# Zilong-Li/BaseVarC

Measured on AMD Instinct MI355X. Metric: sites/sec at N=1e6 samples; achieved HBM GB/s vs roofline, higher is better.
Workload: dtype f64

## Files before the change

### basevarc_amd/csrc/bvc_context.hip

```cpp
#include <cmath>
#include <cstdlib>
#include <cstring>
#include <mutex>
#include <new>

#include "bvc_ctx.h"

hipError_t sync_streams(bvc_ctx *ctx)
{
    hipError_t first = hipSuccess;
    for (hipStream_t s : streams_of(ctx)) {
        const hipError_t e = hipStreamSynchronize(s);
        if (first == hipSuccess) first = e;
    }
    for (bool &p : ctx->em_pending) p = false;
    return first;
}

int drain_on_error(bvc_ctx *ctx, int code)
{
    (void)sync_streams(ctx);
    (void)hipGetLastError();
    return code;
}
// ... 158 lines not shown
    if (hipSetDevice(device) != hipSuccess) { delete ctx; return BVC_ERR_DEVICE; }
    QualLut lut;
    for (int q = 0; q < 128; ++q) {
        const double eps = std::exp(-0.23025850929940458 * q);
        lut.a[q] = 1.0 - eps;
        lut.e[q] = eps / 3.0;
        lut.log_e[q] = std::log(lut.e[q]);
        lut.log_a[q] = std::log(lut.a[q]);
    }
    lut.e_empty = 0.25;
    if (hipMalloc(reinterpret_cast<void **>(&ctx->d_lut), sizeof(QualLut)) != hipSuccess ||
        hipMemcpy(ctx->d_lut, &lut, sizeof(QualLut), hipMemcpyHostToDevice) != hipSuccess) {
        (void)hipGetLastError();
        if (ctx->d_lut) (void)hipFree(ctx->d_lut);
        delete ctx;
        return BVC_ERR_ALLOC;
    }
    int prio_least = 0, prio_greatest = 0;
    if (hipDeviceGetStreamPriorityRange(&prio_least, &prio_greatest) != hipSuccess) { (void)hipGetLastError(); prio_least = 0; }
    const int side_prio = env_int("BVC_SIDE_PRIORITY", 0, 1, 1) ? prio_least : 0;
    bool ok = hipStreamCreateWithFlags(&ctx->own_stream, hipStreamDefault) == hipSuccess &&
              hipEventCreateWithFlags(&ctx->ev_wait, hipEventBlockingSync | hipEventDisableTiming) == hipSuccess &&
              hipStreamCreateWithPriority(&ctx->side, hipStreamNonBlocking, side_prio) == hipSuccess &&
              hipStreamCreateWithPriority(&ctx->side_b, hipStreamNonBlocking, side_prio) == hipSuccess &&
              hipStreamCreateWithPriority(&ctx->side_c, hipStreamNonBlocking, side_prio) == hipSuccess &&
              hipStreamCreateWithFlags(&ctx->copy, hipStreamNonBlocking) == hipSuccess &&
              hipMalloc(reinterpret_cast<void **>(&ctx->d_grp_scratch), kGroupScratchWords * sizeof(int64_t)) == hipSuccess &&
              hipMalloc(reinterpret_cast<void **>(&ctx->d_sink), 256) == hipSuccess;
    for (int b = 0; b < bvc_ctx::kRing && ok; ++b)
        ok = hipEventCreateWithFlags(&ctx->ev_hist_done[b], hipEventDisableTiming) == hipSuccess &&
             hipEventCreateWithFlags(&ctx->ev_em_done[b], hipEventDisableTiming) == hipSuccess;
    for (int b = 0; b < 2 && ok; ++b) ok = hipEventCreateWithFlags(&ctx->ev_upload[b], hipEventDisableTiming) == hipSuccess;
    for (int b = 0; b < 2 && ok; ++b) ok = hipEventCreateWithFlags(&ctx->ev_set_free[b], hipEventDisableTiming) == hipSuccess;
    if (!ok) { (void)hipGetLastError(); bvc_destroy(ctx); return BVC_ERR_DEVICE; }
    ctx->stream = ctx->own_stream;
    *out = ctx;
    return BVC_OK;
}

void *bvc_host_alloc(size_t bytes)
{
    void *p = nullptr;
    if (bytes == 0) bytes = 1;
    if (hipHostMalloc(&p, bytes, hipHostMallocPortable) != hipSuccess) { (void)hipGetLastError(); return nullptr; }
    std::lock_guard<std::mutex> g(g_pinned_mu);
    g_pinned.push_back({static_cast<const char *>(p), bytes});
    return p;
}

void bvc_host_free(void *p)
{
    if (!p) return;
    {
        std::lock_guard<std::mutex> g(g_pinned_mu);
        for (size_t i = 0; i < g_pinned.size(); ++i)
            if (g_pinned[i].first == p) { g_pinned.erase(g_pinned.begin() + (long)i); break; }
    }
    (void)hipHostFree(p);
}

void bvc_destroy(bvc_ctx *ctx)
{
    if (!ctx) return;
    (void)hipSetDevice(ctx->device);
    (void)sync_streams(ctx);
    for (hipStream_t s : {ctx->side, ctx->side_b, ctx->side_c, ctx->copy, ctx->own_stream})
        if (s) (void)hipStreamDestroy(s);
    if (ctx->ev_wait) (void)hipEventDestroy(ctx->ev_wait);
    for (int b = 0; b < bvc_ctx::kRing; ++b) {
        if (ctx->ev_hist_done[b]) (void)hipEventDestroy(ctx->ev_hist_done[b]);
        if (ctx->ev_em_done[b]) (void)hipEventDestroy(ctx->ev_em_done[b]);
    }
    for (int b = 0; b < 2; ++b) {
        if (ctx->ev_upload[b]) (void)hipEventDestroy(ctx->ev_upload[b]);
        if (ctx->ev_set_free[b]) (void)hipEventDestroy(ctx->ev_set_free[b]);
    }
    for (auto &t : ctx->ev_pending) give_back(ctx, t);
    for (auto e : ctx->ev_pool) (void)hipEventDestroy(e);
    if (ctx->d_lut) (void)hipFree(ctx->d_lut);
    if (ctx->d_grp_scratch) (void)hipFree(ctx->d_grp_scratch);
    if (ctx->d_sink) (void)hipFree(ctx->d_sink);
    if (ctx->h_up) (void)hipHostFree(ctx->h_up);
    if (ctx->h_down) (void)hipHostFree(ctx->h_down);
    delete ctx;
}

const char *bvc_last_error(const bvc_ctx *ctx) { return ctx ? ctx->err.c_str() : "null context"; }

int bvc_set_stream(bvc_ctx *ctx, void *hip_stream)
{
    if (!ctx) return BVC_ERR_ARG;
    BVC_HIP(ctx, hipSetDevice(ctx->device));
    BVC_HIP(ctx, sync_streams(ctx));
    ctx->stream = reinterpret_cast<hipStream_t>(hip_stream);
    return BVC_OK;
}

int bvc_synchronize(bvc_ctx *ctx)
{
    if (!ctx) return BVC_ERR_ARG;
    BVC_HIP(ctx, hipSetDevice(ctx->device));
    BVC_HIP(ctx, sync_streams(ctx));
    return BVC_OK;
}

int bvc_set_overlap(bvc_ctx *ctx, int on)
{
    if (!ctx) return BVC_ERR_ARG;
    BVC_HIP(ctx, hipSetDevice(ctx->device));
// ... 100 lines not shown
```

### basevarc_amd/csrc/bvc_ctx.h

```cpp
#pragma once
#include <hip/hip_runtime.h>

#include <array>
#include <cstring>
#include <string>
#include <vector>

#include "bvc_internal.h"

using namespace bvc;

#pragma GCC visibility push(hidden)

struct DevBuf {
    char *p = nullptr;
    size_t cap = 0;
    DevBuf() = default;
    DevBuf(const DevBuf &) = delete;
    DevBuf &operator=(const DevBuf &) = delete;
    ~DevBuf() { if (p) (void)hipFree(p); }
};

struct PileupState {
    DevBuf text, meta, out, called;
// ... 6 lines not shown
        int64_t entries = 0, obs = 0, indels = 0;
        int64_t text_bytes = 0, indel_bytes = 0;
        bool on_device_text = false;
    } tile;
};

struct bvc_ctx {
    int device = -1;
    hipStream_t stream = nullptr;
    hipStream_t own_stream = nullptr;
    hipEvent_t ev_wait = nullptr;
    QualLut *d_lut = nullptr;
    static constexpr int kRing = 4;
    DevBuf d_cnt[kRing];
    bool overlap = false;
    hipStream_t side = nullptr;
    hipStream_t side_b = nullptr, side_c = nullptr;
    unsigned side_flip = 0;
    int flip = 0;
    hipEvent_t ev_hist_done[kRing] = {};
    hipEvent_t ev_em_done[kRing] = {};
    bool em_pending[kRing] = {};
    DevBuf d_grp[kRing];
    DevBuf d_em[kRing + 1];
    DevBuf d_emg[kRing];
    uint32_t *d_sink = nullptr;
    DevBuf d_acc;
    DevBuf d_grp_labels;
    int64_t *d_grp_scratch = nullptr;
    DevBuf d_stage[2];
    hipStream_t copy = nullptr;
    hipEvent_t ev_upload[2] = {nullptr, nullptr};
    hipEvent_t ev_set_free[2] = {nullptr, nullptr};
    PileupState pile;
    char *h_up = nullptr, *h_down = nullptr;
    size_t up_cap = 0, down_cap = 0;
    LaunchState ls;
    bool profiling = false;
    std::vector<hipEvent_t> ev_pool;
    struct Triple { hipEvent_t a, b, c, d; int64_t sites; };
    std::vector<Triple> ev_pending;
    bvc_profile prof{};
    std::string err;
};

struct RingSlot {
    uint32_t *counts = nullptr, *grp = nullptr;
    void *em = nullptr, *emg = nullptr;
};

inline int fail(bvc_ctx *ctx, int code, const char *what, hipError_t e = hipSuccess)
{
    if (ctx) {
        ctx->err = what;
        if (e != hipSuccess) { ctx->err += ": "; ctx->err += hipGetErrorString(e); }
    }
    return code;
}

inline hipError_t wait_stream(bvc_ctx *ctx)
{
    hipError_t e = hipEventRecord(ctx->ev_wait, ctx->stream);
    return e == hipSuccess ? hipEventSynchronize(ctx->ev_wait) : e;
}

#define BVC_HIP(ctx, call)                                                         \
// ... 62 lines not shown
    std::vector<Out> outs;
    explicit PinIO(bvc_ctx *c) : ctx(c) {}
    static size_t al(size_t n) { return (n + 63) & ~(size_t)63; }
    int reserve(size_t up_bytes, size_t down_bytes)
    {
        auto grow = [&](char **buf, size_t *cap, size_t need) -> int {
            if (need <= *cap) return BVC_OK;
            if (*buf) {
                if (wait_stream(ctx) != hipSuccess) return fail(ctx, BVC_ERR_DEVICE, "wait before growing a pinned buffer");
                (void)hipHostFree(*buf);
                *buf = nullptr; *cap = 0;
            }
            const size_t want = need + need / 4 + 4096;
            if (hipHostMalloc(reinterpret_cast<void **>(buf), want, hipHostMallocDefault) != hipSuccess) {
                (void)hipGetLastError();
                return fail(ctx, BVC_ERR_ALLOC, "pinned host allocation failed");
            }
            *cap = want;
            return BVC_OK;
        };
        int rc = grow(&ctx->h_up, &ctx->up_cap, up_bytes);
        return rc == BVC_OK ? grow(&ctx->h_down, &ctx->down_cap, down_bytes) : rc;
    }
    hipError_t h2d(void *dev, const void *host, size_t n)
    {
        if (n == 0) return hipSuccess;
        if (in_pinned(host, n)) return hipMemcpyAsync(dev, host, n, hipMemcpyHostToDevice, ctx->stream);
        if (up_used + n > ctx->up_cap) return hipErrorOutOfMemory;
        char *p = ctx->h_up + up_used;
        std::memcpy(p, host, n);
        up_used += al(n);
        return hipMemcpyAsync(dev, p, n, hipMemcpyHostToDevice, ctx->stream);
    }
    hipError_t d2h(void *host, const void *dev, size_t n)
    {
        if (n == 0) return hipSuccess;
        if (down_used + n > ctx->down_cap) return hipErrorOutOfMemory;
        char *p = ctx->h_down + down_used;
        down_used += al(n);
        outs.push_back(Out{host, p, n});
        return hipMemcpyAsync(p, dev, n, hipMemcpyDeviceToHost, ctx->stream);
    }
    void deliver() { for (auto const &o : outs) std::memcpy(o.dst, o.src, o.n); outs.clear(); }
};

inline int check_common(bvc_ctx *ctx, int64_t n_sites, const void *a, const void *b, const void *c, const void *d)
{
    if (!ctx) return BVC_ERR_ARG;
    if (n_sites < 0) return fail(ctx, BVC_ERR_ARG, "n_sites < 0");
    if (n_sites > 0 && (!a || !b || !c || !d)) return fail(ctx, BVC_ERR_ARG, "null data pointer");
    if (n_sites > (int64_t)0x7FFFFFFF / 64) return fail(ctx, BVC_ERR_ARG, "too many sites in one call (split the tile)");
    BVC_HIP(ctx, hipSetDevice(ctx->device));
    return BVC_OK;
}

inline int check_dense(bvc_ctx *ctx, int64_t n_sites, int64_t n_samples, int64_t row_stride, const void *a, const void *b, const void *c,
                       const void *d)
{
    const int rc = check_common(ctx, n_sites, a, b, c, d);
    if (rc != BVC_OK) return rc;
    return n_samples >= 0 && row_stride >= n_samples ? BVC_OK : fail(ctx, BVC_ERR_ARG, "need 0 <= n_samples <= row_stride");
}

inline int check_offsets_host(bvc_ctx *ctx, int64_t n_sites, const int64_t *offsets)
{
    bool ok = offsets[0] == 0;
    for (int64_t s = 0; s < n_sites && ok; ++s) ok = offsets[s + 1] >= offsets[s];
    return ok ? BVC_OK : fail(ctx, BVC_ERR_ARG, "offsets must start at 0 and be non-decreasing");
}

inline int check_n_groups(bvc_ctx *ctx, int32_t n_groups)
{
    return n_groups >= 1 && n_groups <= BVC_MAX_GROUPS ? BVC_OK : fail(ctx, BVC_ERR_ARG, "n_groups must be 1..32");
// ... 11 lines not shown
```

### basevarc_amd/csrc/bvc_internal.h

```cpp
#pragma once
#include <hip/hip_runtime.h>
#include <stdint.h>

#include <vector>

#include "../../include/bvc.h"

namespace bvc {

struct LaunchState {
    int n_cu = 256;
    int em_waves_per_cu = 0;
    int em_wpb = 4;
    int hist_split = 0;
    int host_chunk_kib = 1 << 19;
    int em_streams = 0;
    int group_pipe = 1;
    int group_log2c = -1;
    int group_big_lds = 1;
    int group_h16 = 0;
    int em_engine = 0;
    int em_tiny_regions = 0;
    int csr_scatter_max = 64;
    int em_prune = 1;
// ... 77 lines not shown
                              int8_t *bases, int8_t *quals, int8_t *ref_base);

struct PileupTile {
    const uint8_t *text = nullptr;
    bool bin = false;
    const uint32_t *line_start = nullptr;
    const int32_t *sample0 = nullptr, *n_in_batch = nullptr;
    int32_t n_batches = 0, n_pos = 0;
    int32_t line_stride = 0;
    const int32_t *n_pos_dev = nullptr;
    int64_t n_lines_cap = 0;
    uint32_t *line_words = nullptr;
    uint32_t *status = nullptr;
    int64_t *entry_off = nullptr, *obs_off = nullptr, *totals = nullptr;
    bvc_pileup_entry *entries = nullptr;
    int32_t *samples = nullptr;
    int8_t *obs_base = nullptr, *obs_qual = nullptr;
    const uint8_t *group_of_sample = nullptr;
    int64_t n_samples = 0;
    int32_t n_groups = 0;
    uint8_t *obs_label = nullptr;
    int32_t *tally = nullptr;
    bvc_pileup_indel *indels = nullptr;
    uint32_t indel_cap = 0;
};
struct bvc_pileup_region { uint32_t start, len, left_src, left_len; };
hipError_t launch_region_carry(hipStream_t stream, const uint8_t *old_text, uint8_t *text, const bvc_pileup_region *regions, int32_t n_batches);
hipError_t launch_region_index(hipStream_t stream, const PileupTile &P, const bvc_pileup_region *regions, const uint32_t *seg_base,
                               int64_t n_segments, uint32_t *seg_nl, int32_t *lines, int32_t max_pos);
hipError_t launch_region_ends(hipStream_t stream, const PileupTile &P, uint32_t *ends);
hipError_t launch_indel_text(hipStream_t stream, const PileupTile &P, uint8_t *dst, uint32_t dst_cap, uint32_t *used);
hipError_t launch_called_scan(hipStream_t stream, const PileupTile &P, const bvc_site_result *results, int64_t *called_off);
hipError_t launch_called_gather(hipStream_t stream, const PileupTile &P, const int64_t *called_off, bvc_pileup_entry *out_entries,
                                int32_t *out_samples);
hipError_t launch_pileup_count(hipStream_t stream, const PileupTile &P);
hipError_t launch_pileup_write(hipStream_t stream, const PileupTile &P, uint32_t carry_in);
hipError_t launch_hist_csr_groups(LaunchState &st, hipStream_t stream, int64_t n_sites, const int64_t *offsets, const int8_t *bases,
                                  const int8_t *quals, const int32_t *sample_of_obs, const uint8_t *group_of_sample, int64_t n_samples,
                                  int n_groups, uint32_t *counts);
hipError_t launch_hist_csr_labels(LaunchState &st, hipStream_t stream, int64_t n_sites, const int64_t *offsets, const uint8_t *obs,
                                  const uint8_t *quals, const uint8_t *group_of_obs, int n_groups, uint32_t *counts);

hipError_t launch_counts_add(hipStream_t stream, int64_t n_words, uint32_t *dst, const uint32_t *src);
hipError_t launch_hist_csr_scatter(const LaunchState &st, hipStream_t stream, int64_t n_sites, const int64_t *offsets, const uint8_t *obs,
                                   const uint8_t *quals, const uint8_t *group_of_obs, int n_groups, int64_t max_len, uint32_t *counts);
hipError_t launch_hist_csr_add(LaunchState &st, hipStream_t stream, int64_t n_sites, const int64_t *offsets, const uint8_t *obs,
                               const uint8_t *quals, const uint8_t *group_of_obs, int n_groups, int64_t min_len, uint32_t *counts);

constexpr int kStatsMaxLog2c = 4;
constexpr int kSiteStatsTrip = 4096;
hipError_t launch_site_stats(LaunchState &st, hipStream_t stream, int64_t n_sites, const int64_t *offsets, const bvc_pileup_entry *entries,
                             const int8_t *ref_base, const bvc_site_result *results, bvc_site_stats *stats);

hipError_t launch_inflate(hipStream_t stream, const uint8_t *comp, const bvc_bgzf_block *blocks, int64_t n_blocks, uint8_t *out, uint32_t *status);

#ifdef BVC_CHECK_LDS
hipError_t debug_read_inflate(uint32_t *out8, bool reset);
hipError_t debug_read_pileup(uint32_t *out8, bool reset);
hipError_t debug_read_site_stats(uint32_t *out8, bool reset);
hipError_t debug_read_hist(uint32_t *out8, bool reset);
hipError_t debug_read_wave_engine(uint32_t *out8, bool reset);
hipError_t debug_read_items(uint32_t *out8, bool reset);
#endif

}
```

### basevarc_amd/csrc/bvc_pileup.hip

```cpp
#include "bvc_ctx.h"

extern "C" {

int bvc_inflate_blocks(bvc_ctx *ctx, const uint8_t *comp, int64_t comp_bytes, const bvc_bgzf_block *blocks, int64_t n_blocks,
                       uint8_t *out, int64_t out_bytes, uint32_t *status, uint32_t flags)
{
    if (!ctx) return BVC_ERR_ARG;
    if (n_blocks < 0 || comp_bytes < 0 || out_bytes < 0) return fail(ctx, BVC_ERR_ARG, "negative size");
    if (n_blocks == 0) return BVC_OK;
    if (!comp || !blocks || !status || (!out && out_bytes > 0)) return fail(ctx, BVC_ERR_ARG, "null data pointer");
    BVC_HIP(ctx, hipSetDevice(ctx->device));
    if (flags & BVC_PTR_DEVICE) {
        BVC_HIP(ctx, launch_inflate(ctx->stream, comp, blocks, n_blocks, out, status));
        return BVC_OK;
    }
    for (int64_t i = 0; i < n_blocks; ++i) {
        const bvc_bgzf_block &b = blocks[i];
        if (b.comp_off < 0 || b.comp_len < 0 || b.comp_off + b.comp_len > comp_bytes || b.isize < 0 || b.isize > 65536 || b.out_off < 0 ||
            b.out_off + b.isize > out_bytes)
            return fail(ctx, BVC_ERR_ARG, "block outside its buffer");
    }
    uint8_t *d_c, *d_o; bvc_bgzf_block *d_b; uint32_t *d_s;
    int rc = carve(ctx, ctx->d_stage[0], 256, [&](Layout &L) {
        d_c = L.take<uint8_t>((size_t)comp_bytes, 16);
// ... 188 lines not shown
            d_reg = L.take<bvc_pileup_region>(nb);
            d_sb = L.take<uint32_t>(nb + 1);
            d_sn = L.take<uint32_t>(segs, 4);
            d_lines = L.take<int32_t>(nb, 4);
            d_ends = L.take<uint32_t>(nb, 4);
        });
    if (rc != BVC_OK) return rc;
    uint8_t *text_out = reinterpret_cast<uint8_t *>(pile.pz_text[nw].p);
    P.text = text_out;
    int32_t *d_T = reinterpret_cast<int32_t *>(reinterpret_cast<char *>(P.status) + 128);
    P.n_pos_dev = d_T;
    PinIO io(ctx);
    rc = io.reserve((n_blocks > 0 && in_pinned(comp, (size_t)comp_bytes) ? 0 : (size_t)comp_bytes) + (size_t)n_blocks * sizeof(bvc_bgzf_block) +
                        nb * (sizeof(bvc_pileup_region) + 12) + 1024,
                    (size_t)n_blocks * 4 + nb * 8 + 1024);
    if (rc != BVC_OK) return rc;
    BVC_HIP_D(ctx, hipMemsetAsync(P.status, 0, clear, ctx->stream));
    std::vector<uint32_t> bst((size_t)n_blocks);
    std::vector<uint32_t> ends(nb);
    uint32_t st[8] = {0, 0, 0, 0, 0, 0, 0, 0};
    int64_t tot[2] = {0, 0};
    int32_t Tgot = 0;
    if (nb > 0) {
        if (n_blocks > 0) {
            BVC_HIP_D(ctx, io.h2d(pile.pz_comp.p, comp, (size_t)comp_bytes));
            BVC_HIP_D(ctx, io.h2d(d_blk, blk.data(), (size_t)n_blocks * sizeof(bvc_bgzf_block)));
        }
        BVC_HIP_D(ctx, io.h2d(d_reg, reg.data(), nb * sizeof(bvc_pileup_region)));
        BVC_HIP_D(ctx, io.h2d(d_sb, seg_base.data(), (nb + 1) * 4));
        BVC_HIP_D(ctx, io.h2d(d_s0, sample0, nb * 4));
        BVC_HIP_D(ctx, io.h2d(d_nib, n_in_batch, nb * 4));
        BVC_HIP_D(ctx, launch_region_carry(ctx->stream, reinterpret_cast<const uint8_t *>(pile.pz_text[pile.pz_cur].p), text_out, d_reg,
                                           n_batches));
        if (n_blocks > 0)
            BVC_HIP_D(ctx, launch_inflate(ctx->stream, reinterpret_cast<const uint8_t *>(pile.pz_comp.p), d_blk, n_blocks, text_out, d_bst));
        BVC_HIP_D(ctx, launch_region_index(ctx->stream, P, d_reg, d_sb, (int64_t)segs, d_sn, d_lines, max_positions));
        BVC_HIP_D(ctx, launch_region_ends(ctx->stream, P, d_ends));
        BVC_HIP_D(ctx, launch_pileup_count(ctx->stream, P));
        if (n_blocks > 0) BVC_HIP_D(ctx, io.d2h(bst.data(), d_bst, (size_t)n_blocks * 4));
        BVC_HIP_D(ctx, io.d2h(lines_of_batch, d_lines, nb * 4));
        BVC_HIP_D(ctx, io.d2h(ends.data(), d_ends, nb * 4));
        BVC_HIP_D(ctx, io.d2h(&Tgot, d_T, 4));
    }
    BVC_HIP_D(ctx, io.d2h(st, P.status, sizeof st));
    BVC_HIP_D(ctx, io.d2h(tot, P.totals, sizeof tot));
    BVC_HIP_D(ctx, wait_stream(ctx));
    io.deliver();
    for (int64_t i = 0; i < n_blocks; ++i)
        if (bst[(size_t)i] != 0) {
            pile.left_len.assign(nb, 0u);
            return fail(ctx, BVC_ERR_DATA, bst[(size_t)i] == 10 ? "a BGZF block of a temp batch fails its CRC32"
                                                                : "a BGZF block of a temp batch is not valid deflate of its ISIZE bytes");
        }
    for (size_t b = 0; b < nb; ++b) { pile.left_src[b] = ends[b]; pile.left_len[b] = region_end[b] - ends[b]; }
    pile.pz_cur = nw;
    P.n_pos = Tgot; P.n_pos_dev = nullptr;
    pile.tile.text_bytes = (int64_t)text_bytes;
    pile.tile.on_device_text = true;
    *n_positions = Tgot;
    if (Tgot == 0) return BVC_OK;
    if (st[0] != 0) return BVC_PILEUP_IRREGULAR;
    pile.tile.entries = tot[0]; pile.tile.obs = tot[1]; pile.tile.indels = st[1]; pile.tile.indel_bytes = st[4];
    pile.tile.begun = true;
    *n_entries = tot[0]; *n_indels = st[1]; *indel_text_bytes = st[4];
    return BVC_OK;
}

int bvc_pileup_text(bvc_ctx *ctx, char *text, int64_t text_cap, int64_t *text_bytes_needed, uint32_t *line_start)
{
    if (!ctx || !text_bytes_needed) return BVC_ERR_ARG;
    const PileupState::Tile &tile = ctx->pile.tile;
    if (!tile.on_device_text) return fail(ctx, BVC_ERR_ARG, "bvc_pileup_text without a tile from bvc_pileup_begin_bgzf");
    *text_bytes_needed = tile.text_bytes;
    if (!text) return BVC_OK;
    if (text_cap < tile.text_bytes || !line_start) return fail(ctx, BVC_ERR_ARG, "text buffer too small / null line table");
    BVC_HIP(ctx, hipSetDevice(ctx->device));
    const PileupTile &P = tile.P;
    if (tile.text_bytes) BVC_HIP(ctx, hipMemcpyAsync(text, P.text, (size_t)tile.text_bytes, hipMemcpyDeviceToHost, ctx->stream));
    if (P.n_batches > 0)
        BVC_HIP(ctx, hipMemcpy2DAsync(line_start, (size_t)(P.n_pos + 1) * 4, P.line_start, (size_t)P.line_stride * 4, (size_t)(P.n_pos + 1) * 4,
                                      (size_t)P.n_batches, hipMemcpyDeviceToHost, ctx->stream));
    BVC_HIP(ctx, wait_stream(ctx));
    return BVC_OK;
}

static int pileup_finish_impl(bvc_ctx *ctx, const int8_t *ref_base, double min_af, const uint8_t carry_in[5], uint8_t carry_out[5],
                              const uint8_t *group_of_sample, int64_t n_samples, int32_t n_groups,
                              int64_t *entry_off, int32_t *tally, int64_t *called_off, int64_t called_cap, bvc_pileup_entry *entries,
                              int32_t *samples, bvc_pileup_indel *indels, char *indel_text, bvc_site_result *results,
                              bvc_group_result *grp_results, bvc_site_stats *stats)
{
    if (!ctx) return BVC_ERR_ARG;
    PileupState &pile = ctx->pile;
    PileupState::Tile &tile = pile.tile;
    if (!tile.begun) return fail(ctx, BVC_ERR_ARG, "bvc_pileup_finish without a bvc_pileup_begin that returned BVC_OK");
    if (tile.on_device_text && tile.indels > 0 && !indel_text) return fail(ctx, BVC_ERR_ARG, "indel_text is needed: the tile's text is on the device only");
    tile.begun = false;
    PileupTile &P = tile.P;
    const int64_t T = P.n_pos, n_e = tile.entries, n_o = tile.obs, n_i = tile.indels, n_it = tile.indel_bytes;
    if (!carry_in || !carry_out || !entry_off) return fail(ctx, BVC_ERR_ARG, "null pointer");
    if (T > 0 && (!ref_base || !tally || !results)) return fail(ctx, BVC_ERR_ARG, "null pointer");
    const bool called_only = called_off != nullptr;
    if ((n_e > 0 && !called_only && (!entries || !samples)) || (n_i > 0 && !indels)) return fail(ctx, BVC_ERR_ARG, "null pointer");
    if (called_only && (called_cap < 0 || (called_cap > 0 && (!entries || !samples)))) return fail(ctx, BVC_ERR_ARG, "null pointer");
    if (n_groups < 0 || n_groups > BVC_MAX_GROUPS) return fail(ctx, BVC_ERR_ARG, "n_groups must be 0..32");
    if (n_groups > 0 && (!grp_results || n_samples < 0 || (n_samples > 0 && !group_of_sample))) return fail(ctx, BVC_ERR_ARG, "null group pointer");
    BVC_HIP(ctx, hipSetDevice(ctx->device));
    int8_t *d_ref; bvc_site_result *d_res; uint8_t *d_g, *d_itext; bvc_group_result *d_gres; int64_t *d_called_off; bvc_site_stats *d_stats;
    int rc = carve(ctx, pile.out, 256, [&](Layout &L) {
        P.entries = L.take<bvc_pileup_entry>((size_t)n_e, 16);
        P.samples = L.take<int32_t>((size_t)n_e, 16);
        P.obs_base = L.take<int8_t>((size_t)n_o, 16);
        P.obs_qual = L.take<int8_t>((size_t)n_o, 16);
        P.obs_label = L.take<uint8_t>((size_t)(n_groups ? n_o : 0), 16);
        P.indels = L.take<bvc_pileup_indel>((size_t)n_i, 16);
        d_ref = L.take<int8_t>((size_t)T, 16);
        d_res = L.take<bvc_site_result>((size_t)T);
        d_g = L.take<uint8_t>((size_t)(n_groups ? n_samples : 0), 16);
        d_gres = L.take<bvc_group_result>((size_t)T * (size_t)n_groups);
        d_itext = L.take<uint8_t>((size_t)(indel_text ? n_it : 0), 16);
        d_called_off = L.take<int64_t>(called_only ? (size_t)(T + 1) : 0);
        d_stats = L.take<bvc_site_stats>(stats ? (size_t)T : 0);
    });
    if (rc != BVC_OK) return rc;
    P.indel_cap = (uint32_t)n_i;
    P.group_of_sample = d_g; P.n_samples = n_groups ? n_samples : 0; P.n_groups = n_groups;
    const uint32_t cin = (uint32_t)(carry_in[0] & 7u) | ((uint32_t)(carry_in[4] & 1u) << 3) | 0x80u | ((uint32_t)carry_in[1] << 8) |
                         ((uint32_t)carry_in[2] << 16) | ((uint32_t)carry_in[3] << 24);
    uint32_t cout = cin;
    PinIO io(ctx);
    rc = io.reserve((size_t)T + (size_t)(n_groups > 0 ? n_samples : 0) + 1024,
                    (size_t)T * (sizeof(bvc_site_result) + 32 * 4 + 8 + (size_t)n_groups * sizeof(bvc_group_result)) +
                        (size_t)(called_only ? 0 : n_e) * (sizeof(bvc_pileup_entry) + 4) + (called_only ? (size_t)(T + 1) * 8 : 0) +
                        (size_t)n_i * sizeof(bvc_pileup_indel) + (size_t)n_it + (stats ? (size_t)T * sizeof(bvc_site_stats) : 0) + 4096);
    if (rc != BVC_OK) return rc;
    if (T > 0) {
        BVC_HIP_D(ctx, io.h2d(d_ref, ref_base, (size_t)T));
        if (n_groups > 0 && n_samples > 0) BVC_HIP_D(ctx, io.h2d(d_g, group_of_sample, (size_t)n_samples));
        if ((int64_t)P.n_pos * P.n_batches > 0) BVC_HIP_D(ctx, launch_pileup_write(ctx->stream, P, cin));
        if (n_groups > 0)
            rc = run_csr_labels_device(ctx, T, P.obs_off, reinterpret_cast<const uint8_t *>(P.obs_base),
                                       reinterpret_cast<const uint8_t *>(P.obs_qual), P.obs_label, d_ref, min_af, n_groups, d_res, d_gres);
        else
            rc = run_csr_device(ctx, T, P.obs_off, P.obs_base, P.obs_qual, d_ref, min_af, nullptr, nullptr, d_res);
        if (rc == BVC_OK) rc = join_side(ctx);
        if (rc != BVC_OK) return drain_on_error(ctx, rc);
        if (stats) BVC_HIP_D(ctx, launch_site_stats(ctx->ls, ctx->stream, T, P.entry_off, P.entries, d_ref, d_res, d_stats));
        BVC_HIP_D(ctx, io.d2h(results, d_res, (size_t)T * sizeof(bvc_site_result)));
        if (stats) BVC_HIP_D(ctx, io.d2h(stats, d_stats, (size_t)T * sizeof(bvc_site_stats)));
        if (n_groups > 0)
            BVC_HIP_D(ctx, io.d2h(grp_results, d_gres, (size_t)T * (size_t)n_groups * sizeof(bvc_group_result)));
        BVC_HIP_D(ctx, io.d2h(tally, P.tally, (size_t)T * 32 * 4));
        if (n_e && !called_only) {
            BVC_HIP_D(ctx, io.d2h(entries, P.entries, (size_t)n_e * sizeof(bvc_pileup_entry)));
            BVC_HIP_D(ctx, io.d2h(samples, P.samples, (size_t)n_e * 4));
        }
        if (called_only) {
            BVC_HIP_D(ctx, launch_called_scan(ctx->stream, P, d_res, d_called_off));
            BVC_HIP_D(ctx, io.d2h(called_off, d_called_off, (size_t)(T + 1) * 8));
        }
        if (n_i && indel_text) {
            BVC_HIP_D(ctx, launch_indel_text(ctx->stream, P, d_itext, (uint32_t)n_it, P.status + 5));
            if (n_it) BVC_HIP_D(ctx, io.d2h(indel_text, d_itext, (size_t)n_it));
        }
        if (n_i) BVC_HIP_D(ctx, io.d2h(indels, P.indels, (size_t)n_i * sizeof(bvc_pileup_indel)));
        if ((int64_t)P.n_pos * P.n_batches > 0) BVC_HIP_D(ctx, io.d2h(&cout, P.status + 3, 4));
    }
    BVC_HIP_D(ctx, io.d2h(entry_off, P.entry_off, (size_t)(T + 1) * 8));
    BVC_HIP_D(ctx, wait_stream(ctx));
    io.deliver();
    if (called_only && T == 0) called_off[0] = 0;
    if (called_only && T > 0 && called_off[T] > 0) {
        const int64_t n_c = called_off[T];
        if (n_c > called_cap) return fail(ctx, BVC_ERR_ARG, "called_cap is smaller than the entries of the called positions (n_entries of the begin call always suffices)");
        bvc_pileup_entry *d_ce; int32_t *d_cs;
        rc = carve(ctx, pile.called, 0, [&](Layout &L) {
            d_ce = L.take<bvc_pileup_entry>((size_t)n_c);
            d_cs = L.take<int32_t>((size_t)n_c);
        });
        if (rc != BVC_OK) return rc;
        io.down_used = 0;
        rc = io.reserve(0, (size_t)n_c * (sizeof(bvc_pileup_entry) + 4) + 4096);
        if (rc != BVC_OK) return rc;
        BVC_HIP_D(ctx, launch_called_gather(ctx->stream, P, d_called_off, d_ce, d_cs));
        BVC_HIP_D(ctx, io.d2h(entries, d_ce, (size_t)n_c * sizeof(bvc_pileup_entry)));
        BVC_HIP_D(ctx, io.d2h(samples, d_cs, (size_t)n_c * 4));
        BVC_HIP_D(ctx, wait_stream(ctx));
        io.deliver();
    }
    carry_out[0] = (uint8_t)(cout & 7u); carry_out[1] = (uint8_t)(cout >> 8); carry_out[2] = (uint8_t)(cout >> 16);
    carry_out[3] = (uint8_t)(cout >> 24); carry_out[4] = (uint8_t)((cout >> 3) & 1u);
    return BVC_OK;
}

int bvc_pileup_finish(bvc_ctx *ctx, const int8_t *ref_base, double min_af, const uint8_t carry_in[5], uint8_t carry_out[5],
                      const uint8_t *group_of_sample, int64_t n_samples, int32_t n_groups,
                      int64_t *entry_off, int32_t *tally, bvc_pileup_entry *entries, int32_t *samples,
                      bvc_pileup_indel *indels, char *indel_text, bvc_site_result *results, bvc_group_result *grp_results)
{
    return pileup_finish_impl(ctx, ref_base, min_af, carry_in, carry_out, group_of_sample, n_samples, n_groups, entry_off, tally, nullptr, 0,
                              entries, samples, indels, indel_text, results, grp_results, nullptr);
}

int bvc_pileup_finish_called(bvc_ctx *ctx, const int8_t *ref_base, double min_af, const uint8_t carry_in[5], uint8_t carry_out[5],
                             const uint8_t *group_of_sample, int64_t n_samples, int32_t n_groups,
                             int64_t *entry_off, int32_t *tally, int64_t *called_off, int64_t called_cap, bvc_pileup_entry *entries,
                             int32_t *samples, bvc_pileup_indel *indels, char *indel_text, bvc_site_result *results,
                             bvc_group_result *grp_results)
{
    if (ctx && !called_off) return fail(ctx, BVC_ERR_ARG, "null pointer");
    return pileup_finish_impl(ctx, ref_base, min_af, carry_in, carry_out, group_of_sample, n_samples, n_groups, entry_off, tally, called_off,
                              called_cap, entries, samples, indels, indel_text, results, grp_results, nullptr);
}

int bvc_pileup_finish_called_stats(bvc_ctx *ctx, const int8_t *ref_base, double min_af, const uint8_t carry_in[5], uint8_t carry_out[5],
                                   const uint8_t *group_of_sample, int64_t n_samples, int32_t n_groups,
                                   int64_t *entry_off, int32_t *tally, int64_t *called_off, int64_t called_cap, bvc_pileup_entry *entries,
                                   int32_t *samples, bvc_pileup_indel *indels, char *indel_text, bvc_site_result *results,
                                   bvc_group_result *grp_results, bvc_site_stats *stats)
{
    if (ctx && !called_off) return fail(ctx, BVC_ERR_ARG, "null pointer");
// ... 6 lines not shown
```

### basevarc_amd/csrc/inflate_kernel.hip

```cpp
#include <hip/hip_runtime.h>

#ifndef BVC_INFLATE_WINDOW
#define BVC_INFLATE_WINDOW 4096
#endif

#include "bvc_device.h"
#include "bvc_internal.h"

namespace bvc {
namespace {

constexpr uint32_t kWinBytes = BVC_INFLATE_WINDOW, kWinMask = kWinBytes - 1;
constexpr uint32_t kDump = kWinBytes;
constexpr bool kWholeWindow = kWinBytes == 32768;
static_assert((kWinBytes & kWinMask) == 0 && kWinBytes >= 4096 && kWinBytes <= 32768, "the LDS ring: a power of two, 4..32 KiB");
constexpr int kLitBits = 9, kDistBits = 7, kPreBits = 7;
constexpr uint32_t kValid = 0x80000000u;
constexpr uint32_t kKindLiteral = 0u << 24, kKindEnd = 1u << 24, kKindLength = 2u << 24, kKindBad = 3u << 24, kKindMask = 3u << 24;

__device__ const uint16_t kLenBase[29] = {3, 4, 5, 6, 7, 8, 9, 10, 11, 13, 15, 17, 19, 23, 27, 31, 35, 43, 51, 59, 67, 83, 99, 115, 131, 163, 195, 227, 258};
__device__ const uint8_t kLenExtra[29] = {0, 0, 0, 0, 0, 0, 0, 0, 1, 1, 1, 1, 2, 2, 2, 2, 3, 3, 3, 3, 4, 4, 4, 4, 5, 5, 5, 5, 0};
__device__ const uint16_t kDistBase[30] = {1, 2, 3, 4, 5, 7, 9, 13, 17, 25, 33, 49, 65, 97, 129, 193, 257, 385, 513, 769, 1025, 1537, 2049, 3073, 4097, 6145,
                                           8193, 12289, 16385, 24577};
__device__ const uint8_t kDistExtra[30] = {0, 0, 0, 0, 1, 1, 2, 2, 3, 3, 4, 4, 5, 5, 6, 6, 7, 7, 8, 8, 9, 9, 10, 10, 11, 11, 12, 12, 13, 13};
// ... 577 lines not shown
        const uint32_t n = (uint32_t)blocks[blk].isize;
        const uint64_t base = o0 & ~(uint64_t)15;
        const uint32_t span = (uint32_t)(o0 - base) + n;
        const uint32_t per = ((span + kWave - 1) / kWave + 15u) & ~15u;
        const uint64_t lo64 = base + (uint64_t)per * (uint32_t)lane, hi64 = lo64 + per;
        const uint64_t lo = lo64 < o0 ? o0 : (lo64 > o0 + n ? o0 + n : lo64), hi = hi64 < o0 ? o0 : (hi64 > o0 + n ? o0 + n : hi64);
        uint32_t c = 0xFFFFFFFFu;
        uint64_t at = lo;
        while (at < hi && (at & 15u)) { c = tab[(c ^ out[at]) & 255u] ^ (c >> 8); ++at; }
        for (; at + 16 <= hi; at += 16) {
            const uint4 v = *reinterpret_cast<const uint4 *>(out + at);
            const uint32_t w[4] = {v.x, v.y, v.z, v.w};
#pragma unroll
            for (int j = 0; j < 4; ++j)
#pragma unroll
                for (int b = 0; b < 4; ++b) c = tab[(c ^ (w[j] >> (8 * b))) & 255u] ^ (c >> 8);
        }
        for (; at < hi; ++at) c = tab[(c ^ out[at]) & 255u] ^ (c >> 8);
        const uint32_t mine = ~c;
        const uint32_t len = (uint32_t)(hi - lo);
        const uint32_t op_full = crc_shift_op(per);
        uint32_t acc = (uint32_t)__builtin_amdgcn_readlane((int)mine, 0);
        for (int k = 1; k < kWave; ++k) {
            const uint32_t lk = (uint32_t)__shfl((int)len, k, kWave), ck = (uint32_t)__shfl((int)mine, k, kWave);
            if (lk == 0u) continue;
            acc = crc_multmodp(lk == per ? op_full : crc_shift_op(lk), acc) ^ ck;
        }
        if (lane == 0 && acc != blocks[blk].crc32) status[blk] = kErrCrc;
    }
}

}

hipError_t launch_inflate(hipStream_t stream, const uint8_t *comp, const bvc_bgzf_block *blocks, int64_t n_blocks, uint8_t *out, uint32_t *status)
{
    if (n_blocks <= 0) return hipSuccess;
    hipLaunchKernelGGL(inflate_kernel, dim3((unsigned)(n_blocks < 65536 ? n_blocks : 65536)), dim3(kWave), 0, stream, comp, blocks, n_blocks, out, status);
    hipLaunchKernelGGL(crc32_kernel, dim3((unsigned)(n_blocks < 65536 ? n_blocks : 65536)), dim3(kWave), 0, stream, blocks, n_blocks, out, status);
    return hipGetLastError();
}

#ifdef BVC_CHECK_LDS
BVC_DEFINE_DEBUG_READER(debug_read_inflate)
#endif

}
```

### basevarc_amd/csrc/pileup_kernel.hip

```cpp
#include <hip/hip_runtime.h>

#include "bvc_device.h"
#include "bvc_internal.h"

namespace bvc {
namespace {

constexpr int kParseWaves = 4;
constexpr uint32_t kTokValid = 0x80u;

typedef uint32_t u32x4 __attribute__((ext_vector_type(4)));
typedef uint32_t u32x2 __attribute__((ext_vector_type(2)));

__device__ __forceinline__ uint32_t wave_incl_scan(uint32_t v, int lane)
{
#pragma unroll
    for (int d = 1; d < kWave; d <<= 1) {
        const uint32_t u = (uint32_t)__shfl_up((int)v, d, kWave);
        if (lane >= d) v += u;
    }
    return v;
}

__device__ __forceinline__ uint32_t wave_sum(uint32_t v)
// ... 707 lines not shown
    }
}

__global__ __launch_bounds__(1024) void called_scan_kernel(int64_t n_pos, const bvc_site_result *__restrict__ results,
                                                           const int64_t *__restrict__ entry_off, int64_t *__restrict__ called_off)
{
    __shared__ int64_t wave_sum[16];
    __shared__ int64_t running;
    const int lane = threadIdx.x & (kWave - 1), wave = threadIdx.x >> 6;
    if (threadIdx.x == 0) running = 0;
    __syncthreads();
    for (int64_t t0 = 0; t0 < n_pos; t0 += 1024) {
        const int64_t t = t0 + threadIdx.x;
        const int64_t mine = (t < n_pos && results[t].called) ? entry_off[t + 1] - entry_off[t] : 0;
        int64_t incl = mine;
        for (int d = 1; d < kWave; d <<= 1) {
            const int64_t up = __shfl_up(incl, d);
            if (lane >= d) incl += up;
        }
        if (lane == kWave - 1) wave_sum[wave] = incl;
        __syncthreads();
        int64_t before = running;
        for (int w = 0; w < wave; ++w) before += wave_sum[w];
        if (t < n_pos) called_off[t] = before + incl - mine;
        __syncthreads();
        if (threadIdx.x == 1023) running = before + incl;
        __syncthreads();
    }
    if (threadIdx.x == 0) called_off[n_pos] = running;
}

__global__ void called_gather_kernel(int64_t n_pos, const int64_t *__restrict__ entry_off, const int64_t *__restrict__ called_off,
                                     const bvc_pileup_entry *__restrict__ entries, const int32_t *__restrict__ samples,
                                     bvc_pileup_entry *__restrict__ out_entries, int32_t *__restrict__ out_samples)
{
    for (int64_t t = blockIdx.x; t < n_pos; t += gridDim.x) {
        const int64_t at = called_off[t], n = called_off[t + 1] - at, from = entry_off[t];
        for (int64_t i = threadIdx.x; i < n; i += blockDim.x) {
            out_entries[at + i] = entries[from + i];
            out_samples[at + i] = samples[from + i];
        }
    }
}

hipError_t launch_called_scan(hipStream_t stream, const PileupTile &P, const bvc_site_result *results, int64_t *called_off)
{
    hipLaunchKernelGGL(called_scan_kernel, dim3(1), dim3(1024), 0, stream, (int64_t)P.n_pos, results, P.entry_off, called_off);
    return hipGetLastError();
}

hipError_t launch_called_gather(hipStream_t stream, const PileupTile &P, const int64_t *called_off, bvc_pileup_entry *out_entries,
                                int32_t *out_samples)
{
    if (P.n_pos <= 0) return hipSuccess;
    hipLaunchKernelGGL(called_gather_kernel, dim3((unsigned)(P.n_pos < 16384 ? P.n_pos : 16384)), dim3(256), 0, stream, (int64_t)P.n_pos,
                       P.entry_off, called_off, P.entries, P.samples, out_entries, out_samples);
    return hipGetLastError();
}

hipError_t launch_region_carry(hipStream_t stream, const uint8_t *old_text, uint8_t *text, const bvc_pileup_region *regions, int32_t n_batches)
{
    if (n_batches <= 0) return hipSuccess;
    hipLaunchKernelGGL(region_carry_kernel, dim3((unsigned)n_batches), dim3(256), 0, stream, old_text, text, regions);
    return hipGetLastError();
}

hipError_t launch_region_index(hipStream_t stream, const PileupTile &P, const bvc_pileup_region *regions, const uint32_t *seg_base,
                               int64_t n_segments, uint32_t *seg_nl, int32_t *lines, int32_t max_pos)
{
    if (P.n_batches <= 0) return hipSuccess;
    RegionArgs A{};
    A.text = P.text; A.regions = regions; A.seg_base = seg_base; A.n_batches = P.n_batches; A.max_pos = max_pos; A.line_stride = P.line_stride;
    A.seg_nl = seg_nl; A.lines = lines; A.n_pos = const_cast<int32_t *>(P.n_pos_dev); A.line_start = const_cast<uint32_t *>(P.line_start);
    const int64_t blocks = (n_segments + kParseWaves - 1) / kParseWaves;
    const unsigned grid = (unsigned)(blocks < 65536 ? (blocks > 0 ? blocks : 1) : 65536);
    hipLaunchKernelGGL(region_lines_kernel<false>, dim3(grid), dim3(kParseWaves * kWave), 0, stream, A);
    hipLaunchKernelGGL(region_scan_kernel, dim3((unsigned)P.n_batches), dim3(kWave), 0, stream, A);
    hipLaunchKernelGGL(region_lines_kernel<true>, dim3(grid), dim3(kParseWaves * kWave), 0, stream, A);
    return hipGetLastError();
}

__global__ void region_ends_kernel(const uint32_t *__restrict__ line_start, int32_t line_stride, const int32_t *__restrict__ n_pos, int32_t n_batches,
                                   uint32_t *__restrict__ ends)
{
    const int b = blockIdx.x * blockDim.x + threadIdx.x;
    if (b < n_batches) ends[b] = line_start[(int64_t)b * line_stride + *n_pos];
}

hipError_t launch_region_ends(hipStream_t stream, const PileupTile &P, uint32_t *ends)
// ... 73 lines not shown
```

Baseline: 3.359 million.

## Overlap CRC check on copy stream and speculatively gather called entries early

Splits inflate and CRC32 into separate launches and runs the CRC kernel on the copy stream, so it overlaps with region indexing and pileup counting. The main stream waits on a CRC event only before the status readback. The called-entry gather now runs in the first device pass, and a speculative prefix of the gathered entries (a fixed share of n_entries) is copied back with the first batch of readbacks. The second sync-and-copy round trip is only needed when more entries are called than fit in that prefix. This costs an up-front allocation sized to called_cap, and the gather kernel must bail out when the total exceeds capacity.

```diff
diff --git a/basevarc_amd/csrc/bvc_context.hip b/basevarc_amd/csrc/bvc_context.hip
--- a/basevarc_amd/csrc/bvc_context.hip
+++ b/basevarc_amd/csrc/bvc_context.hip
@@ -214,6 +214,8 @@
              hipEventCreateWithFlags(&ctx->ev_em_done[b], hipEventDisableTiming) == hipSuccess;
     for (int b = 0; b < 2 && ok; ++b) ok = hipEventCreateWithFlags(&ctx->ev_upload[b], hipEventDisableTiming) == hipSuccess;
     for (int b = 0; b < 2 && ok; ++b) ok = hipEventCreateWithFlags(&ctx->ev_set_free[b], hipEventDisableTiming) == hipSuccess;
+    ok = ok && hipEventCreateWithFlags(&ctx->ev_inflated, hipEventDisableTiming) == hipSuccess &&
+         hipEventCreateWithFlags(&ctx->ev_crc, hipEventDisableTiming) == hipSuccess;
     if (!ok) { (void)hipGetLastError(); bvc_destroy(ctx); return BVC_ERR_DEVICE; }
     ctx->stream = ctx->own_stream;
     *out = ctx;
@@ -257,6 +259,8 @@
         if (ctx->ev_upload[b]) (void)hipEventDestroy(ctx->ev_upload[b]);
         if (ctx->ev_set_free[b]) (void)hipEventDestroy(ctx->ev_set_free[b]);
     }
+    if (ctx->ev_inflated) (void)hipEventDestroy(ctx->ev_inflated);
+    if (ctx->ev_crc) (void)hipEventDestroy(ctx->ev_crc);
     for (auto &t : ctx->ev_pending) give_back(ctx, t);
     for (auto e : ctx->ev_pool) (void)hipEventDestroy(e);
     if (ctx->d_lut) (void)hipFree(ctx->d_lut);
diff --git a/basevarc_amd/csrc/bvc_ctx.h b/basevarc_amd/csrc/bvc_ctx.h
--- a/basevarc_amd/csrc/bvc_ctx.h
+++ b/basevarc_amd/csrc/bvc_ctx.h
@@ -62,6 +62,7 @@
     hipStream_t copy = nullptr;
     hipEvent_t ev_upload[2] = {nullptr, nullptr};
     hipEvent_t ev_set_free[2] = {nullptr, nullptr};
+    hipEvent_t ev_inflated = nullptr, ev_crc = nullptr;
     PileupState pile;
     char *h_up = nullptr, *h_down = nullptr;
     size_t up_cap = 0, down_cap = 0;
@@ -190,13 +191,14 @@
         up_used += al(n);
         return hipMemcpyAsync(dev, p, n, hipMemcpyHostToDevice, ctx->stream);
     }
-    hipError_t d2h(void *host, const void *dev, size_t n)
+    hipError_t d2h(void *host, const void *dev, size_t n, const char **held = nullptr)
     {
         if (n == 0) return hipSuccess;
         if (down_used + n > ctx->down_cap) return hipErrorOutOfMemory;
         char *p = ctx->h_down + down_used;
         down_used += al(n);
-        outs.push_back(Out{host, p, n});
+        if (held) *held = p;
+        else outs.push_back(Out{host, p, n});
         return hipMemcpyAsync(p, dev, n, hipMemcpyDeviceToHost, ctx->stream);
     }
     void deliver() { for (auto const &o : outs) std::memcpy(o.dst, o.src, o.n); outs.clear(); }
diff --git a/basevarc_amd/csrc/bvc_internal.h b/basevarc_amd/csrc/bvc_internal.h
--- a/basevarc_amd/csrc/bvc_internal.h
+++ b/basevarc_amd/csrc/bvc_internal.h
@@ -133,7 +133,7 @@
 hipError_t launch_indel_text(hipStream_t stream, const PileupTile &P, uint8_t *dst, uint32_t dst_cap, uint32_t *used);
 hipError_t launch_called_scan(hipStream_t stream, const PileupTile &P, const bvc_site_result *results, int64_t *called_off);
 hipError_t launch_called_gather(hipStream_t stream, const PileupTile &P, const int64_t *called_off, bvc_pileup_entry *out_entries,
-                                int32_t *out_samples);
+                                int32_t *out_samples, int64_t cap);
 hipError_t launch_pileup_count(hipStream_t stream, const PileupTile &P);
 hipError_t launch_pileup_write(hipStream_t stream, const PileupTile &P, uint32_t carry_in);
 hipError_t launch_hist_csr_groups(LaunchState &st, hipStream_t stream, int64_t n_sites, const int64_t *offsets, const int8_t *bases,
@@ -154,6 +154,8 @@
                              const int8_t *ref_base, const bvc_site_result *results, bvc_site_stats *stats);
 
 hipError_t launch_inflate(hipStream_t stream, const uint8_t *comp, const bvc_bgzf_block *blocks, int64_t n_blocks, uint8_t *out, uint32_t *status);
+hipError_t launch_inflate_only(hipStream_t stream, const uint8_t *comp, const bvc_bgzf_block *blocks, int64_t n_blocks, uint8_t *out, uint32_t *status);
+hipError_t launch_crc32(hipStream_t stream, const bvc_bgzf_block *blocks, int64_t n_blocks, const uint8_t *out, uint32_t *status);
 
 #ifdef BVC_CHECK_LDS
 hipError_t debug_read_inflate(uint32_t *out8, bool reset);
diff --git a/basevarc_amd/csrc/bvc_pileup.hip b/basevarc_amd/csrc/bvc_pileup.hip
--- a/basevarc_amd/csrc/bvc_pileup.hip
+++ b/basevarc_amd/csrc/bvc_pileup.hip
@@ -244,11 +244,17 @@
         BVC_HIP_D(ctx, io.h2d(d_nib, n_in_batch, nb * 4));
         BVC_HIP_D(ctx, launch_region_carry(ctx->stream, reinterpret_cast<const uint8_t *>(pile.pz_text[pile.pz_cur].p), text_out, d_reg,
                                            n_batches));
-        if (n_blocks > 0)
-            BVC_HIP_D(ctx, launch_inflate(ctx->stream, reinterpret_cast<const uint8_t *>(pile.pz_comp.p), d_blk, n_blocks, text_out, d_bst));
+        if (n_blocks > 0) {
+            BVC_HIP_D(ctx, launch_inflate_only(ctx->stream, reinterpret_cast<const uint8_t *>(pile.pz_comp.p), d_blk, n_blocks, text_out, d_bst));
+            BVC_HIP_D(ctx, hipEventRecord(ctx->ev_inflated, ctx->stream));
+            BVC_HIP_D(ctx, hipStreamWaitEvent(ctx->copy, ctx->ev_inflated, 0));
+            BVC_HIP_D(ctx, launch_crc32(ctx->copy, d_blk, n_blocks, text_out, d_bst));
+            BVC_HIP_D(ctx, hipEventRecord(ctx->ev_crc, ctx->copy));
+        }
         BVC_HIP_D(ctx, launch_region_index(ctx->stream, P, d_reg, d_sb, (int64_t)segs, d_sn, d_lines, max_positions));
         BVC_HIP_D(ctx, launch_region_ends(ctx->stream, P, d_ends));
         BVC_HIP_D(ctx, launch_pileup_count(ctx->stream, P));
+        if (n_blocks > 0) BVC_HIP_D(ctx, hipStreamWaitEvent(ctx->stream, ctx->ev_crc, 0));
         if (n_blocks > 0) BVC_HIP_D(ctx, io.d2h(bst.data(), d_bst, (size_t)n_blocks * 4));
         BVC_HIP_D(ctx, io.d2h(lines_of_batch, d_lines, nb * 4));
         BVC_HIP_D(ctx, io.d2h(ends.data(), d_ends, nb * 4));
@@ -295,6 +301,8 @@
     BVC_HIP(ctx, wait_stream(ctx));
     return BVC_OK;
 }
+
+static int64_t called_share(int64_t n_entries) { return n_entries / 16 > 4096 ? n_entries / 16 : 4096; }
 
 static int pileup_finish_impl(bvc_ctx *ctx, const int8_t *ref_base, double min_af, const uint8_t carry_in[5], uint8_t carry_out[5],
                               const uint8_t *group_of_sample, int64_t n_samples, int32_t n_groups,
@@ -319,7 +327,15 @@
     if (n_groups > 0 && (!grp_results || n_samples < 0 || (n_samples > 0 && !group_of_sample))) return fail(ctx, BVC_ERR_ARG, "null group pointer");
     BVC_HIP(ctx, hipSetDevice(ctx->device));
     int8_t *d_ref; bvc_site_result *d_res; uint8_t *d_g, *d_itext; bvc_group_result *d_gres; int64_t *d_called_off; bvc_site_stats *d_stats;
-    int rc = carve(ctx, pile.out, 256, [&](Layout &L) {
+    const int64_t n_room = called_only && T > 0 ? (called_cap < n_e ? called_cap : n_e) : 0;
+    const int64_t n_spec = n_room < called_share(n_e) ? n_room : called_share(n_e);
+    bvc_pileup_entry *d_ce = nullptr; int32_t *d_cs = nullptr;
+    int rc = carve(ctx, pile.called, 0, [&](Layout &L) {
+        d_ce = L.take<bvc_pileup_entry>((size_t)n_room);
+        d_cs = L.take<int32_t>((size_t)n_room);
+    });
+    if (rc != BVC_OK) return rc;
+    rc = carve(ctx, pile.out, 256, [&](Layout &L) {
         P.entries = L.take<bvc_pileup_entry>((size_t)n_e, 16);
         P.samples = L.take<int32_t>((size_t)n_e, 16);
         P.obs_base = L.take<int8_t>((size_t)n_o, 16);
@@ -340,10 +356,11 @@
     const uint32_t cin = (uint32_t)(carry_in[0] & 7u) | ((uint32_t)(carry_in[4] & 1u) << 3) | 0x80u | ((uint32_t)carry_in[1] << 8) |
                          ((uint32_t)carry_in[2] << 16) | ((uint32_t)carry_in[3] << 24);
     uint32_t cout = cin;
+    const char *h_ce = nullptr, *h_cs = nullptr;
     PinIO io(ctx);
     rc = io.reserve((size_t)T + (size_t)(n_groups > 0 ? n_samples : 0) + 1024,
                     (size_t)T * (sizeof(bvc_site_result) + 32 * 4 + 8 + (size_t)n_groups * sizeof(bvc_group_result)) +
-                        (size_t)(called_only ? 0 : n_e) * (sizeof(bvc_pileup_entry) + 4) + (called_only ? (size_t)(T + 1) * 8 : 0) +
+                        (size_t)(called_only ? n_spec : n_e) * (sizeof(bvc_pileup_entry) + 4) + (called_only ? (size_t)(T + 1) * 8 : 0) +
                         (size_t)n_i * sizeof(bvc_pileup_indel) + (size_t)n_it + (stats ? (size_t)T * sizeof(bvc_site_stats) : 0) + 4096);
     if (rc != BVC_OK) return rc;
     if (T > 0) {
@@ -370,6 +387,11 @@
         if (called_only) {
             BVC_HIP_D(ctx, launch_called_scan(ctx->stream, P, d_res, d_called_off));
             BVC_HIP_D(ctx, io.d2h(called_off, d_called_off, (size_t)(T + 1) * 8));
+            if (n_room > 0) {
+                BVC_HIP_D(ctx, launch_called_gather(ctx->stream, P, d_called_off, d_ce, d_cs, n_room));
+                BVC_HIP_D(ctx, io.d2h(nullptr, d_ce, (size_t)n_spec * sizeof(bvc_pileup_entry), &h_ce));
+                BVC_HIP_D(ctx, io.d2h(nullptr, d_cs, (size_t)n_spec * 4, &h_cs));
+            }
         }
         if (n_i && indel_text) {
             BVC_HIP_D(ctx, launch_indel_text(ctx->stream, P, d_itext, (uint32_t)n_it, P.status + 5));
@@ -385,20 +407,18 @@
     if (called_only && T > 0 && called_off[T] > 0) {
         const int64_t n_c = called_off[T];
         if (n_c > called_cap) return fail(ctx, BVC_ERR_ARG, "called_cap is smaller than the entries of the called positions (n_entries of the begin call always suffices)");
-        bvc_pileup_entry *d_ce; int32_t *d_cs;
-        rc = carve(ctx, pile.called, 0, [&](Layout &L) {
-            d_ce = L.take<bvc_pileup_entry>((size_t)n_c);
-            d_cs = L.take<int32_t>((size_t)n_c);
-        });
-        if (rc != BVC_OK) return rc;
-        io.down_used = 0;
-        rc = io.reserve(0, (size_t)n_c * (sizeof(bvc_pileup_entry) + 4) + 4096);
-        if (rc != BVC_OK) return rc;
-        BVC_HIP_D(ctx, launch_called_gather(ctx->stream, P, d_called_off, d_ce, d_cs));
-        BVC_HIP_D(ctx, io.d2h(entries, d_ce, (size_t)n_c * sizeof(bvc_pileup_entry)));
-        BVC_HIP_D(ctx, io.d2h(samples, d_cs, (size_t)n_c * 4));
-        BVC_HIP_D(ctx, wait_stream(ctx));
-        io.deliver();
+        const int64_t n_here = n_c < n_spec ? n_c : n_spec;
+        std::memcpy(entries, h_ce, (size_t)n_here * sizeof(bvc_pileup_entry));
+        std::memcpy(samples, h_cs, (size_t)n_here * 4);
+        if (n_c > n_spec) {
+            io.down_used = 0;
+            rc = io.reserve(0, (size_t)(n_c - n_spec) * (sizeof(bvc_pileup_entry) + 4) + 4096);
+            if (rc != BVC_OK) return rc;
+            BVC_HIP_D(ctx, io.d2h(entries + n_spec, d_ce + n_spec, (size_t)(n_c - n_spec) * sizeof(bvc_pileup_entry)));
+            BVC_HIP_D(ctx, io.d2h(samples + n_spec, d_cs + n_spec, (size_t)(n_c - n_spec) * 4));
+            BVC_HIP_D(ctx, wait_stream(ctx));
+            io.deliver();
+        }
     }
     carry_out[0] = (uint8_t)(cout & 7u); carry_out[1] = (uint8_t)(cout >> 8); carry_out[2] = (uint8_t)(cout >> 16);
     carry_out[3] = (uint8_t)(cout >> 24); carry_out[4] = (uint8_t)((cout >> 3) & 1u);
diff --git a/basevarc_amd/csrc/inflate_kernel.hip b/basevarc_amd/csrc/inflate_kernel.hip
--- a/basevarc_amd/csrc/inflate_kernel.hip
+++ b/basevarc_amd/csrc/inflate_kernel.hip
@@ -633,12 +633,24 @@
 
 }
 
-hipError_t launch_inflate(hipStream_t stream, const uint8_t *comp, const bvc_bgzf_block *blocks, int64_t n_blocks, uint8_t *out, uint32_t *status)
+hipError_t launch_inflate_only(hipStream_t stream, const uint8_t *comp, const bvc_bgzf_block *blocks, int64_t n_blocks, uint8_t *out, uint32_t *status)
 {
     if (n_blocks <= 0) return hipSuccess;
     hipLaunchKernelGGL(inflate_kernel, dim3((unsigned)(n_blocks < 65536 ? n_blocks : 65536)), dim3(kWave), 0, stream, comp, blocks, n_blocks, out, status);
+    return hipGetLastError();
+}
+
+hipError_t launch_crc32(hipStream_t stream, const bvc_bgzf_block *blocks, int64_t n_blocks, const uint8_t *out, uint32_t *status)
+{
+    if (n_blocks <= 0) return hipSuccess;
     hipLaunchKernelGGL(crc32_kernel, dim3((unsigned)(n_blocks < 65536 ? n_blocks : 65536)), dim3(kWave), 0, stream, blocks, n_blocks, out, status);
     return hipGetLastError();
+}
+
+hipError_t launch_inflate(hipStream_t stream, const uint8_t *comp, const bvc_bgzf_block *blocks, int64_t n_blocks, uint8_t *out, uint32_t *status)
+{
+    const hipError_t e = launch_inflate_only(stream, comp, blocks, n_blocks, out, status);
+    return e == hipSuccess ? launch_crc32(stream, blocks, n_blocks, out, status) : e;
 }
 
 #ifdef BVC_CHECK_LDS
diff --git a/basevarc_amd/csrc/pileup_kernel.hip b/basevarc_amd/csrc/pileup_kernel.hip
--- a/basevarc_amd/csrc/pileup_kernel.hip
+++ b/basevarc_amd/csrc/pileup_kernel.hip
@@ -763,8 +763,9 @@
 
 __global__ void called_gather_kernel(int64_t n_pos, const int64_t *__restrict__ entry_off, const int64_t *__restrict__ called_off,
                                      const bvc_pileup_entry *__restrict__ entries, const int32_t *__restrict__ samples,
-                                     bvc_pileup_entry *__restrict__ out_entries, int32_t *__restrict__ out_samples)
-{
+                                     bvc_pileup_entry *__restrict__ out_entries, int32_t *__restrict__ out_samples, int64_t cap)
+{
+    if (called_off[n_pos] > cap) return;
     for (int64_t t = blockIdx.x; t < n_pos; t += gridDim.x) {
         const int64_t at = called_off[t], n = called_off[t + 1] - at, from = entry_off[t];
         for (int64_t i = threadIdx.x; i < n; i += blockDim.x) {
@@ -781,11 +782,11 @@
 }
 
 hipError_t launch_called_gather(hipStream_t stream, const PileupTile &P, const int64_t *called_off, bvc_pileup_entry *out_entries,
-                                int32_t *out_samples)
+                                int32_t *out_samples, int64_t cap)
 {
     if (P.n_pos <= 0) return hipSuccess;
     hipLaunchKernelGGL(called_gather_kernel, dim3((unsigned)(P.n_pos < 16384 ? P.n_pos : 16384)), dim3(256), 0, stream, (int64_t)P.n_pos,
-                       P.entry_off, called_off, P.entries, P.samples, out_entries, out_samples);
+                       P.entry_off, called_off, P.entries, P.samples, out_entries, out_samples, cap);
     return hipGetLastError();
 }
 
```

Result: no change. 3.372 million (median of 3 runs) (+0.4%).
